# lucasbrynte/gasfm

Hardware: AMD Instinct MI355X
Metric: GAT-stack edges/sec (fwd+bwd) on cam/point scene graph; 1/2/4/8 MI355X (higher is better)
Workload: dtype fp32; 1 GPU; config 4: m=1000 cameras, n=200000 points, E=4001638 projections, 12-block GraphAttnSfMNet (learning_euc widths) fwd+bwd; cameras=1000, points=200000, edges=4001638, blocks=12, parallelism=single GPU

## Files before the change

### gasfm_amd/csrc/global_attn.hip

```cpp
#include <hip/hip_runtime.h>

#include <cstdint>

#include "common.hpp"

namespace gasfm {
namespace {

constexpr int kT = 256;
constexpr int H = 4;
#ifndef GASFM_GATT_CHUNK_V
#define GASFM_GATT_CHUNK_V 8
#endif
#ifndef GASFM_GATT_CHUNK_P
#define GASFM_GATT_CHUNK_P 256
#endif
constexpr int kChunkV = GASFM_GATT_CHUNK_V;
constexpr int kChunkP = GASFM_GATT_CHUNK_P;
constexpr int kMaxProb = 2;
constexpr int kGroup = 32;

struct GaProb {
  const float* XL;
  int64_t ldXL;
  const int32_t* src;
  const float* XR;
  const float* att;
  const float* bias;
  float* out;
  float* smax;
  float* ssum;
  float* part;
  const float* gout;
  float* dXL;
  int64_t ldDXL;
  float* dXR;
  float* datt;
  float* slots;
  uint32_t* cnt;
  int64_t sl;
  int S, HC, C, blk0, nblk;
  float* gslots;
  uint32_t* gcnt;
  int ngroups;
};
struct GaArgs {
  GaProb p[kMaxProb];
  int nprob;
  float slope;
};

__device__ __forceinline__ float leaky(float z, float slope) { return z > 0.f ? z : z * slope; }

__device__ __forceinline__ float wave_sum(float v) {
#pragma unroll
  for (int o = 32; o > 0; o >>= 1) v += __shfl_xor(v, o);
  return v;
}
__device__ __forceinline__ float wave_max(float v) {
#pragma unroll
  for (int o = 32; o > 0; o >>= 1) v = fmaxf(v, __shfl_xor(v, o));
  return v;
}

__device__ __forceinline__ int find_prob(const GaArgs& a) {
  return (a.nprob > 1 && int(blockIdx.x) >= a.p[1].blk0) ? 1 : 0;
}

__device__ __forceinline__ int src_row(const GaProb& p, int j) { return p.src ? p.src[j] : j; }

__device__ __forceinline__ void st_sc1(float* q, float v) {
  __hip_atomic_store(q, v, __ATOMIC_RELAXED, __HIP_MEMORY_SCOPE_AGENT);
}

__device__ __forceinline__ bool last_arrival(uint32_t* cnt, int n, uint32_t* flag) {
  asm volatile("s_waitcnt vmcnt(0)" ::: "memory");
  __syncthreads();
  if (threadIdx.x == 0) {
    const uint32_t t = __hip_atomic_fetch_add(cnt, 1u, __ATOMIC_RELAXED, __HIP_MEMORY_SCOPE_AGENT);
    *flag = t == uint32_t(n - 1) ? 1u : 0u;
  }
  __syncthreads();
  if (*flag == 0u) return false;
  __builtin_amdgcn_fence(__ATOMIC_ACQUIRE, "agent");
  return true;
}

__device__ void merge_fwd(const GaProb& p, float* sc) {
  __shared__ float MH[H], SH[H];
  __shared__ float accg[4][64];
  const int64_t L = p.sl;
  const int n = p.nblk;
  {
    const int h = threadIdx.x & 3;
    float m = -INFINITY;
    for (int k = threadIdx.x >> 2; k < n; k += kT / 4) m = fmaxf(m, p.slots[int64_t(k) * L + p.HC + h]);
#pragma unroll
    for (int o = 32; o >= 4; o >>= 1) m = fmaxf(m, __shfl_xor(m, o));
    __syncthreads();
    if ((threadIdx.x & 63) < 4) sc[(threadIdx.x >> 6) * 4 + h] = m;
    __syncthreads();
    if (threadIdx.x < H)
      MH[threadIdx.x] = fmaxf(fmaxf(sc[threadIdx.x], sc[4 + threadIdx.x]), fmaxf(sc[8 + threadIdx.x], sc[12 + threadIdx.x]));
    __syncthreads();
  }
  {
    const int h = threadIdx.x & 3;
    const float M = MH[h];
    float s = 0.f;
    for (int k = threadIdx.x >> 2; k < n; k += kT / 4) {
      const float* q = p.slots + int64_t(k) * L + p.HC;
      const float mk = q[h], sk = q[H + h];
      s += mk == -INFINITY ? 0.f : sk * __expf(mk - M);
    }
#pragma unroll
    for (int o = 32; o >= 4; o >>= 1) s += __shfl_xor(s, o);
    __syncthreads();
    if ((threadIdx.x & 63) < 4) sc[(threadIdx.x >> 6) * 4 + h] = s;
    __syncthreads();
    if (threadIdx.x < H)
      SH[threadIdx.x] = (sc[threadIdx.x] + sc[4 + threadIdx.x]) + (sc[8 + threadIdx.x] + sc[12 + threadIdx.x]);
    __syncthreads();
  }
  auto finish = [&](int f, float a) {
    const int h = f / p.C;
    if (p.part) {
      st_sc1(p.part + f, a);
      if (f < H) {
        st_sc1(p.part + p.HC + f, MH[f]);
        st_sc1(p.part + p.HC + H + f, SH[f]);
      }
    } else {
      p.out[f] = a / (SH[h] + 1e-16f) + p.bias[f];
      if (f < H) {
        p.smax[f] = MH[f];
        p.ssum[f] = SH[f];
      }
    }
  };
  if (p.C == 256) {
    const int f0 = 4 * threadIdx.x, h = f0 / 256;
    float4 a = make_float4(0.f, 0.f, 0.f, 0.f);
#pragma unroll 8
    for (int k = 0; k < n; ++k) {
      const float* q = p.slots + int64_t(k) * L;
      const float mk = q[p.HC + h];
      const float w = mk == -INFINITY ? 0.f : __expf(mk - MH[h]);
      const float4 v = *reinterpret_cast<const float4*>(q + f0);
      a.x = fmaf(v.x, w, a.x);
      a.y = fmaf(v.y, w, a.y);
      a.z = fmaf(v.z, w, a.z);
      a.w = fmaf(v.w, w, a.w);
    }
    finish(f0, a.x);
    finish(f0 + 1, a.y);
    finish(f0 + 2, a.z);
    finish(f0 + 3, a.w);
  } else {
    const int f = threadIdx.x & 63, grp = threadIdx.x >> 6, h = f / p.C;
    float a = 0.f;
    if (f < p.HC)
#pragma unroll 8
      for (int k = grp; k < n; k += 4) {
        const float* q = p.slots + int64_t(k) * L;
        const float mk = q[p.HC + h];
        a = fmaf(q[f], mk == -INFINITY ? 0.f : __expf(mk - MH[h]), a);
      }
    accg[grp][f] = a;
    __syncthreads();
    if (threadIdx.x < p.HC) finish(threadIdx.x, (accg[0][f] + accg[1][f]) + (accg[2][f] + accg[3][f]));
  }
}

__device__ void done_fwd(const GaProb& p, int blk, uint32_t* flag, float* sc) {
  if (p.ngroups <= 1) {
    if (last_arrival(p.cnt, p.nblk, flag)) {
      merge_fwd(p, sc);
      if (threadIdx.x == 0) __hip_atomic_store(p.cnt, 0u, __ATOMIC_RELAXED, __HIP_MEMORY_SCOPE_AGENT);
    }
    return;
  }
  const int g = blk / kGroup, n0 = g * kGroup;
  const int ng = p.nblk - n0 < kGroup ? p.nblk - n0 : kGroup;
  if (!last_arrival(p.gcnt + g, ng, flag)) return;
  GaProb q = p;
  q.slots = p.slots + int64_t(n0) * p.sl;
  q.nblk = ng;
  q.part = p.gslots + int64_t(g) * p.sl;
  merge_fwd(q, sc);
  if (threadIdx.x == 0) __hip_atomic_store(p.gcnt + g, 0u, __ATOMIC_RELAXED, __HIP_MEMORY_SCOPE_AGENT);
  __syncthreads();
  if (!last_arrival(p.cnt, p.ngroups, flag)) return;
  GaProb r = p;
  r.slots = p.gslots;
  r.nblk = p.ngroups;
  merge_fwd(r, sc);
  if (threadIdx.x == 0) __hip_atomic_store(p.cnt, 0u, __ATOMIC_RELAXED, __HIP_MEMORY_SCOPE_AGENT);
}

__device__ void fwd_views(const GaProb& p, int blk, float slope, uint32_t* flag, float* sc) {
  const int lane = threadIdx.x & 63, wave = threadIdx.x >> 6;
  const int f0 = 4 * threadIdx.x;
  const int j0 = blk * kChunkV, j1 = min(p.S, j0 + kChunkV);
  const float4 xr = *reinterpret_cast<const float4*>(p.XR + f0);
  const float4 at = *reinterpret_cast<const float4*>(p.att + f0);
  float m = -INFINITY, s = 0.f;
  float4 acc = make_float4(0.f, 0.f, 0.f, 0.f);
  float4 nx = make_float4(0.f, 0.f, 0.f, 0.f);
  if (j0 < j1) nx = *reinterpret_cast<const float4*>(p.XL + int64_t(src_row(p, j0)) * p.ldXL + f0);
  for (int j = j0; j < j1; ++j) {
    const float4 x = nx;
    const int jn = j + 1 < j1 ? j + 1 : j;
    nx = *reinterpret_cast<const float4*>(p.XL + int64_t(src_row(p, jn)) * p.ldXL + f0);
    float e = leaky(x.x + xr.x, slope) * at.x + leaky(x.y + xr.y, slope) * at.y + leaky(x.z + xr.z, slope) * at.z +
              leaky(x.w + xr.w, slope) * at.w;
    e = wave_sum(e);
    const float mn = fmaxf(m, e);
    const float sc0 = m == -INFINITY ? 0.f : __expf(m - mn), w = __expf(e - mn);
    s = fmaf(s, sc0, w);
    acc = make_float4(fmaf(acc.x, sc0, w * x.x), fmaf(acc.y, sc0, w * x.y), fmaf(acc.z, sc0, w * x.z),
                      fmaf(acc.w, sc0, w * x.w));
    m = mn;
  }
  float* slot = p.slots + int64_t(blk) * (p.HC + 2 * H);
  st_sc1(slot + f0, acc.x);
  st_sc1(slot + f0 + 1, acc.y);
  st_sc1(slot + f0 + 2, acc.z);
  st_sc1(slot + f0 + 3, acc.w);
  if (lane == 0) {
    st_sc1(slot + p.HC + wave, m);
    st_sc1(slot + p.HC + H + wave, s);
  }
  done_fwd(p, blk, flag, sc);
}

__device__ void fwd_points(const GaProb& p, int blk, float slope, uint32_t* flag, float* sc) {
  __shared__ float SM[16][H], SS[16][H];
  __shared__ float4 SA[16][16];
  const int ql = threadIdx.x >> 4, fq = threadIdx.x & 15, h = fq >> 2;
  const int f0 = 4 * fq;
  const int j0 = blk * kChunkP, j1 = min(p.S, j0 + kChunkP);
  const float4 xr = *reinterpret_cast<const float4*>(p.XR + f0);
  const float4 at = *reinterpret_cast<const float4*>(p.att + f0);
  float m = -INFINITY, s = 0.f;
  float4 acc = make_float4(0.f, 0.f, 0.f, 0.f);
  constexpr int U = 4;
  for (int jb = j0 + ql; jb < j1; jb += 16 * U) {
    float4 x[U];
#pragma unroll
    for (int u = 0; u < U; ++u) {
      const int j = jb + 16 * u;
      x[u] = *reinterpret_cast<const float4*>(p.XL + int64_t(src_row(p, j < j1 ? j : jb)) * p.ldXL + f0);
    }
#pragma unroll
    for (int u = 0; u < U; ++u) {
      float e = leaky(x[u].x + xr.x, slope) * at.x + leaky(x[u].y + xr.y, slope) * at.y +
                leaky(x[u].z + xr.z, slope) * at.z + leaky(x[u].w + xr.w, slope) * at.w;
      e += __shfl_xor(e, 1);
      e += __shfl_xor(e, 2);
      if (jb + 16 * u < j1) {
        const float mn = fmaxf(m, e);
        const float sc0 = m == -INFINITY ? 0.f : __expf(m - mn), w = __expf(e - mn);
        s = fmaf(s, sc0, w);
        acc = make_float4(fmaf(acc.x, sc0, w * x[u].x), fmaf(acc.y, sc0, w * x[u].y), fmaf(acc.z, sc0, w * x[u].z),
                          fmaf(acc.w, sc0, w * x[u].w));
        m = mn;
      }
    }
  }
  if ((fq & 3) == 0) {
    SM[ql][h] = m;
    SS[ql][h] = s;
  }
  SA[ql][fq] = acc;
  __syncthreads();
  float* slot = p.slots + int64_t(blk) * (p.HC + 2 * H);
  if (threadIdx.x < 16) {
    const int hh = threadIdx.x >> 2;
    float M = -INFINITY;
#pragma unroll
    for (int q = 0; q < 16; ++q) M = fmaxf(M, SM[q][hh]);
    float S = 0.f;
    float4 A = make_float4(0.f, 0.f, 0.f, 0.f);
#pragma unroll
    for (int q = 0; q < 16; ++q) {
      const float mq = SM[q][hh];
      const float w = mq == -INFINITY ? 0.f : __expf(mq - M);
      S = fmaf(SS[q][hh], w, S);
      const float4 a = SA[q][threadIdx.x];
      A = make_float4(fmaf(a.x, w, A.x), fmaf(a.y, w, A.y), fmaf(a.z, w, A.z), fmaf(a.w, w, A.w));
    }
    const int g0 = 4 * threadIdx.x;
    st_sc1(slot + g0, A.x);
    st_sc1(slot + g0 + 1, A.y);
    st_sc1(slot + g0 + 2, A.z);
    st_sc1(slot + g0 + 3, A.w);
    if ((threadIdx.x & 3) == 0) {
      st_sc1(slot + p.HC + hh, M);
      st_sc1(slot + p.HC + H + hh, S);
    }
  }
  done_fwd(p, blk, flag, sc);
}

__global__ __launch_bounds__(kT) void gatt_fwd_kernel(GaArgs a) {
  __shared__ uint32_t flag;
  __shared__ float sc[16];
  const int pi = find_prob(a);
  const GaProb& p = a.p[pi];
  const int blk = int(blockIdx.x) - p.blk0;
  if (p.C == 256)
    fwd_views(p, blk, a.slope, &flag, sc);
  else
    fwd_points(p, blk, a.slope, &flag, sc);
}

__device__ void merge_bwd(const GaProb& p, bool final = true, float* grow = nullptr) {
  __shared__ float acc4[4][2 * 64];
  const int L = 2 * p.HC, n = p.nblk;
  if (p.C == 256) {
    for (int half = 0; half < 2; ++half) {
      const int f0 = 4 * threadIdx.x;
      float4 a = make_float4(0.f, 0.f, 0.f, 0.f);
#pragma unroll 8
      for (int k = 0; k < n; ++k) {
        const float4 v = *reinterpret_cast<const float4*>(p.slots + int64_t(k) * L + half * p.HC + f0);
        a.x += v.x;
        a.y += v.y;
        a.z += v.z;
        a.w += v.w;
      }
      if (!final) {
        float* d = grow + half * p.HC + f0;
        st_sc1(d, a.x);
        st_sc1(d + 1, a.y);
        st_sc1(d + 2, a.z);
        st_sc1(d + 3, a.w);
        continue;
      }
      float* d = half ? p.datt : p.dXR;
      d[f0] = a.x;
      d[f0 + 1] = a.y;
      d[f0 + 2] = a.z;
      d[f0 + 3] = a.w;
    }
    if (final)
      *reinterpret_cast<float4*>(p.datt + p.HC + 4 * threadIdx.x) =
          *reinterpret_cast<const float4*>(p.gout + 4 * threadIdx.x);
  } else {
    const int grp = threadIdx.x >> 6;
#pragma unroll
    for (int r = 0; r < 2; ++r) {
      const int v = (threadIdx.x & 63) + 64 * r;
      float a = 0.f;
      if (v < L)
#pragma unroll 8
        for (int k = grp; k < n; k += 4) a += p.slots[int64_t(k) * L + v];
      acc4[grp][v] = a;
    }
    __syncthreads();
    if (threadIdx.x < L) {
      const float a = (acc4[0][threadIdx.x] + acc4[1][threadIdx.x]) + (acc4[2][threadIdx.x] + acc4[3][threadIdx.x]);
      if (!final)
        st_sc1(grow + threadIdx.x, a);
      else if (threadIdx.x < p.HC)
        p.dXR[threadIdx.x] = a;
      else
        p.datt[threadIdx.x - p.HC] = a;
    }
    if (final && threadIdx.x < p.HC) p.datt[p.HC + threadIdx.x] = p.gout[threadIdx.x];
  }
}

__device__ void done_bwd(const GaProb& p, int blk, uint32_t* flag) {
  if (p.ngroups <= 1) {
    if (last_arrival(p.cnt, p.nblk, flag)) {
      merge_bwd(p);
      if (threadIdx.x == 0) __hip_atomic_store(p.cnt, 0u, __ATOMIC_RELAXED, __HIP_MEMORY_SCOPE_AGENT);
    }
    return;
  }
  const int g = blk / kGroup, n0 = g * kGroup;
  const int ng = p.nblk - n0 < kGroup ? p.nblk - n0 : kGroup;
  if (!last_arrival(p.gcnt + g, ng, flag)) return;
  const int64_t L = 2 * int64_t(p.HC);
  GaProb q = p;
  q.slots = p.slots + int64_t(n0) * L;
  q.nblk = ng;
  merge_bwd(q, false, p.gslots + int64_t(g) * L);
  if (threadIdx.x == 0) __hip_atomic_store(p.gcnt + g, 0u, __ATOMIC_RELAXED, __HIP_MEMORY_SCOPE_AGENT);
  __syncthreads();
  if (!last_arrival(p.cnt, p.ngroups, flag)) return;
  GaProb r = p;
  r.slots = p.gslots;
  r.nblk = p.ngroups;
  merge_bwd(r);
  if (threadIdx.x == 0) __hip_atomic_store(p.cnt, 0u, __ATOMIC_RELAXED, __HIP_MEMORY_SCOPE_AGENT);
}

__device__ void bwd_views(const GaProb& p, int blk, float slope, uint32_t* flag) {
  const int lane = threadIdx.x & 63, wave = threadIdx.x >> 6;
  const int f0 = 4 * threadIdx.x;
  const int j0 = blk * kChunkV, j1 = min(p.S, j0 + kChunkV);
  const float4 xr = *reinterpret_cast<const float4*>(p.XR + f0);
  const float4 at = *reinterpret_cast<const float4*>(p.att + f0);
  const float4 go = *reinterpret_cast<const float4*>(p.gout + f0);
  const float4 o4 = *reinterpret_cast<const float4*>(p.out + f0);
  const float4 b4 = *reinterpret_cast<const float4*>(p.bias + f0);
  const float M = p.smax[wave], inv = 1.f / (p.ssum[wave] + 1e-16f);
  const float delta =
      wave_sum(go.x * (o4.x - b4.x) + go.y * (o4.y - b4.y) + go.z * (o4.z - b4.z) + go.w * (o4.w - b4.w));
  float4 dxr = make_float4(0.f, 0.f, 0.f, 0.f), dat = dxr;
  int jr = 0;
  float4 nx = make_float4(0.f, 0.f, 0.f, 0.f);
  if (j0 < j1) {
    jr = src_row(p, j0);
    nx = *reinterpret_cast<const float4*>(p.XL + int64_t(jr) * p.ldXL + f0);
  }
  for (int j = j0; j < j1; ++j) {
    const float4 x = nx;
    const int row = jr;
    const int jn = j + 1 < j1 ? j + 1 : j;
    jr = src_row(p, jn);
    nx = *reinterpret_cast<const float4*>(p.XL + int64_t(jr) * p.ldXL + f0);
    const float z[4] = {x.x + xr.x, x.y + xr.y, x.z + xr.z, x.w + xr.w};
    const float a4[4] = {at.x, at.y, at.z, at.w};
    const float g4[4] = {go.x, go.y, go.z, go.w};
    const float xv[4] = {x.x, x.y, x.z, x.w};
    float e = 0.f, da = 0.f;
#pragma unroll
    for (int k = 0; k < 4; ++k) {
      e = fmaf(leaky(z[k], slope), a4[k], e);
      da = fmaf(g4[k], xv[k], da);
    }
    e = wave_sum(e);
    da = wave_sum(da);
    const float alpha = __expf(e - M) * inv;
    const float de = alpha * (da - delta);
    float dxl[4], dz[4];
#pragma unroll
    for (int k = 0; k < 4; ++k) {
      dz[k] = de * a4[k] * (z[k] > 0.f ? 1.f : slope);
      dxl[k] = fmaf(alpha, g4[k], dz[k]);
    }
    *reinterpret_cast<float4*>(p.dXL + int64_t(row) * p.ldDXL + f0) = make_float4(dxl[0], dxl[1], dxl[2], dxl[3]);
    dxr = make_float4(dxr.x + dz[0], dxr.y + dz[1], dxr.z + dz[2], dxr.w + dz[3]);
    dat = make_float4(fmaf(de, leaky(z[0], slope), dat.x), fmaf(de, leaky(z[1], slope), dat.y),
                      fmaf(de, leaky(z[2], slope), dat.z), fmaf(de, leaky(z[3], slope), dat.w));
  }
  float* slot = p.slots + int64_t(blk) * 2 * p.HC;
  st_sc1(slot + f0, dxr.x);
  st_sc1(slot + f0 + 1, dxr.y);
  st_sc1(slot + f0 + 2, dxr.z);
  st_sc1(slot + f0 + 3, dxr.w);
  st_sc1(slot + p.HC + f0, dat.x);
  st_sc1(slot + p.HC + f0 + 1, dat.y);
  st_sc1(slot + p.HC + f0 + 2, dat.z);
  st_sc1(slot + p.HC + f0 + 3, dat.w);
  (void)lane;
  done_bwd(p, blk, flag);
}

__device__ void bwd_points(const GaProb& p, int blk, float slope, uint32_t* flag) {
  __shared__ float4 SX[16][16], SD[16][16];
  const int ql = threadIdx.x >> 4, fq = threadIdx.x & 15, h = fq >> 2;
  const int f0 = 4 * fq;
  const int j0 = blk * kChunkP, j1 = min(p.S, j0 + kChunkP);
  const float4 xr = *reinterpret_cast<const float4*>(p.XR + f0);
  const float4 at = *reinterpret_cast<const float4*>(p.att + f0);
  const float4 go = *reinterpret_cast<const float4*>(p.gout + f0);
  const float4 o4 = *reinterpret_cast<const float4*>(p.out + f0);
  const float4 b4 = *reinterpret_cast<const float4*>(p.bias + f0);
  const float M = p.smax[h], inv = 1.f / (p.ssum[h] + 1e-16f);
  float delta = go.x * (o4.x - b4.x) + go.y * (o4.y - b4.y) + go.z * (o4.z - b4.z) + go.w * (o4.w - b4.w);
  delta += __shfl_xor(delta, 1);
  delta += __shfl_xor(delta, 2);
  const float a4[4] = {at.x, at.y, at.z, at.w};
  const float g4[4] = {go.x, go.y, go.z, go.w};
  float4 dxr = make_float4(0.f, 0.f, 0.f, 0.f), dat = dxr;
  constexpr int U = 4;
  for (int jb = j0 + ql; jb < j1; jb += 16 * U) {
    float4 x[U];
    int rows[U];
#pragma unroll
    for (int u = 0; u < U; ++u) {
      const int j = jb + 16 * u;
      rows[u] = src_row(p, j < j1 ? j : jb);
      x[u] = *reinterpret_cast<const float4*>(p.XL + int64_t(rows[u]) * p.ldXL + f0);
    }
#pragma unroll
    for (int u = 0; u < U; ++u) {
      const float xv[4] = {x[u].x, x[u].y, x[u].z, x[u].w};
      float z[4], e = 0.f, da = 0.f;
#pragma unroll
      for (int k = 0; k < 4; ++k) {
        z[k] = xv[k] + (k == 0 ? xr.x : k == 1 ? xr.y : k == 2 ? xr.z : xr.w);
        e = fmaf(leaky(z[k], slope), a4[k], e);
        da = fmaf(g4[k], xv[k], da);
      }
      e += __shfl_xor(e, 1);
      e += __shfl_xor(e, 2);
      da += __shfl_xor(da, 1);
      da += __shfl_xor(da, 2);
      if (jb + 16 * u < j1) {
        const float alpha = __expf(e - M) * inv;
        const float de = alpha * (da - delta);
        float dxl[4];
#pragma unroll
        for (int k = 0; k < 4; ++k) {
          const float dz = de * a4[k] * (z[k] > 0.f ? 1.f : slope);
          dxl[k] = fmaf(alpha, g4[k], dz);
          if (k == 0) dxr.x += dz, dat.x = fmaf(de, leaky(z[k], slope), dat.x);
          if (k == 1) dxr.y += dz, dat.y = fmaf(de, leaky(z[k], slope), dat.y);
          if (k == 2) dxr.z += dz, dat.z = fmaf(de, leaky(z[k], slope), dat.z);
          if (k == 3) dxr.w += dz, dat.w = fmaf(de, leaky(z[k], slope), dat.w);
        }
        *reinterpret_cast<float4*>(p.dXL + int64_t(rows[u]) * p.ldDXL + f0) =
            make_float4(dxl[0], dxl[1], dxl[2], dxl[3]);
      }
    }
  }
  SX[ql][fq] = dxr;
  SD[ql][fq] = dat;
  __syncthreads();
  float* slot = p.slots + int64_t(blk) * 2 * p.HC;
  if (threadIdx.x < 32) {
    const int q = threadIdx.x & 15, half = threadIdx.x >> 4;
    float4 sum = make_float4(0.f, 0.f, 0.f, 0.f);
#pragma unroll
    for (int l = 0; l < 16; ++l) {
      const float4 v = half ? SD[l][q] : SX[l][q];
      sum = make_float4(sum.x + v.x, sum.y + v.y, sum.z + v.z, sum.w + v.w);
    }
    float* d = slot + half * p.HC + 4 * q;
    st_sc1(d, sum.x);
    st_sc1(d + 1, sum.y);
    st_sc1(d + 2, sum.z);
    st_sc1(d + 3, sum.w);
  }
  done_bwd(p, blk, flag);
}

__global__ __launch_bounds__(kT) void gatt_bwd_kernel(GaArgs a) {
  __shared__ uint32_t flag;
  const int pi = find_prob(a);
  const GaProb& p = a.p[pi];
  const int blk = int(blockIdx.x) - p.blk0;
  if (p.C == 256)
    bwd_views(p, blk, a.slope, &flag);
  else
    bwd_points(p, blk, a.slope, &flag);
}

struct Unpack {
  const float* G;
  int64_t blk, roff, soff, ld_dst;
  float* rows_dst;
  float* sum_dst;
  int W, chunk, width, m, sn;
};

__device__ __forceinline__ int unpack_units(const Unpack& u) {
  return (u.rows_dst ? u.m * (u.width / 4) : 0) + (u.sum_dst ? u.sn / 4 : 0);
}

__device__ __forceinline__ void unpack_unit(const Unpack& u, int k) {
  const int nr = u.rows_dst ? u.m * (u.width / 4) : 0;
  if (k < nr) {
    const int w4 = u.width / 4, c = k / w4, q = k % w4;
    const float4 v = *reinterpret_cast<const float4*>(u.G + int64_t(c / u.chunk) * u.blk + u.roff +
                                                      int64_t(c % u.chunk) * u.width + 4 * q);
    *reinterpret_cast<float4*>(u.rows_dst + int64_t(c) * u.ld_dst + 4 * q) = v;
    return;
  }
  const int j = k - nr;
  float4 acc = *reinterpret_cast<const float4*>(u.G + u.soff + 4 * j);
  for (int r = 1; r < u.W; ++r) {
    const float4 v = *reinterpret_cast<const float4*>(u.G + int64_t(r) * u.blk + u.soff + 4 * j);
    acc = make_float4(acc.x + v.x, acc.y + v.y, acc.z + v.z, acc.w + v.w);
  }
  *reinterpret_cast<float4*>(u.sum_dst + 4 * j) = acc;
}

__global__ __launch_bounds__(kT) void exchange_unpack_kernel(Unpack u) {
  const int k = int(blockIdx.x) * kT + int(threadIdx.x);
  if (k < unpack_units(u)) unpack_unit(u, k);
}

__global__ __launch_bounds__(kT) void gatt_merge_kernel(GaArgs a, Unpack u) {
  __shared__ float sc[16];
  if (int(blockIdx.x) < a.nprob) {
    merge_fwd(a.p[blockIdx.x], sc);
    return;
  }
  const int k = (int(blockIdx.x) - a.nprob) * kT + int(threadIdx.x);
  if (k < unpack_units(u)) unpack_unit(u, k);
}

int chunk_of(int C) { return C == 256 ? kChunkV : kChunkP; }

int groups_of(int nblk) { return nblk > kGroup ? (nblk + kGroup - 1) / kGroup : 1; }

int setup(const gasfm_gatt_prob* in, int nprob, float* scratch, uint32_t* counters, bool bwd, GaArgs& a) {
  a.nprob = nprob;
  int blocks = 0;
  float* ws = scratch;
  uint32_t* cn = counters;
  for (int q = 0; q < nprob; ++q) {
    const gasfm_gatt_prob& s = in[q];
    GaProb& p = a.p[q];
    p.XL = s.XL, p.ldXL = s.ldXL, p.src = s.src, p.XR = s.XR, p.att = s.att, p.bias = s.bias;
    p.out = s.out, p.smax = s.smax, p.ssum = s.ssum, p.part = s.part;
    p.gout = s.gout, p.dXL = s.dXL, p.ldDXL = s.ldDXL, p.dXR = s.dXR, p.datt = s.datt;
    p.S = s.S, p.HC = s.HC, p.C = s.HC / H;
    p.nblk = (s.S + chunk_of(p.C) - 1) / chunk_of(p.C);
    if (p.nblk < 1) p.nblk = 1;
    p.blk0 = blocks;
    p.slots = ws;
    p.sl = p.HC + 2 * H;
    const int64_t slot = bwd ? 2 * p.HC : p.HC + 2 * H;
    ws += int64_t(p.nblk) * slot;
    p.ngroups = groups_of(p.nblk);
    p.gslots = ws;
    if (p.ngroups > 1) ws += int64_t(p.ngroups) * slot;
    p.cnt = cn++;
    p.gcnt = cn;
    if (p.ngroups > 1) cn += p.ngroups;
    blocks += p.nblk;
  }
  for (int q = nprob; q < kMaxProb; ++q) a.p[q].blk0 = blocks;
  return blocks;
}

}
}

using namespace gasfm;

static int gatt_check(int32_t nprob, const gasfm_gatt_prob* probs, bool bwd) {
  GASFM_REQUIRE(nprob >= 1 && nprob <= kMaxProb && probs, "gasfm_gatt: nprob=%d", nprob);
  for (int q = 0; q < nprob; ++q) {
    const gasfm_gatt_prob& p = probs[q];
    GASFM_REQUIRE(p.HC == 4 * 256 || p.HC == 4 * 16, "gasfm_gatt: problem %d HC=%d (H = 4, C in {16, 256})", q, p.HC);
    GASFM_REQUIRE(p.S >= 0 && (p.XL || p.S == 0) && p.XR && p.att && p.bias && p.ldXL % 4 == 0 && (p.ldXL >= p.HC || p.S == 0),
                  "gasfm_gatt: problem %d S=%d / pointers / ldXL", q, p.S);
    GASFM_REQUIRE(aligned16(p.XL) && aligned16(p.XR) && aligned16(p.att) && aligned16(p.bias),
                  "gasfm_gatt: problem %d alignment", q);
    if (!bwd) {
      GASFM_REQUIRE(p.part || (p.out && p.smax && p.ssum), "gasfm_gatt_fwd: problem %d outputs", q);
    } else {
      GASFM_REQUIRE(p.gout && p.out && p.smax && p.ssum && (p.dXL || p.S == 0) && p.dXR && p.datt && p.ldDXL % 4 == 0 &&
                        (aligned16(p.dXL) || p.S == 0) && aligned16(p.gout) && aligned16(p.out) && aligned16(p.datt),
                    "gasfm_gatt_bwd: problem %d pointers", q);
    }
  }
  return GASFM_OK;
}

static int64_t nblk_of(const gasfm_gatt_prob& p) {
  const int C = p.HC / H;
  const int64_t nblk = (p.S + chunk_of(C) - 1) / chunk_of(C);
  return nblk < 1 ? 1 : nblk;
}

extern "C" int64_t gasfm_gatt_scratch_floats(int32_t nprob, const gasfm_gatt_prob* probs) {
  int64_t n = 0;
  for (int q = 0; q < nprob; ++q) {
    const int64_t nblk = nblk_of(probs[q]), ng = groups_of(int(nblk));
    n += (nblk + (ng > 1 ? ng : 0)) * (2 * int64_t(probs[q].HC) + 2 * H);
  }
  return n + 16;
}

extern "C" int32_t gasfm_gatt_counters(int32_t nprob, const gasfm_gatt_prob* probs) {
  int32_t n = 0;
  for (int q = 0; q < nprob; ++q) {
    const int ng = groups_of(int(nblk_of(probs[q])));
    n += 1 + (ng > 1 ? ng : 0);
  }
  return n;
}

extern "C" int gasfm_gatt_fwd(int32_t nprob, const gasfm_gatt_prob* probs, float slope, float* scratch,
                              uint32_t* counters, void* stream) {
  const int s0 = gatt_check(nprob, probs, false);
  if (s0 != GASFM_OK) return s0;
  GASFM_REQUIRE(scratch && counters, "gasfm_gatt_fwd: scratch / counters");
  GaArgs a{};
  a.slope = slope;
  const int blocks = setup(probs, nprob, scratch, counters, false, a);
  hipLaunchKernelGGL(gatt_fwd_kernel, dim3(blocks), dim3(kT), 0, reinterpret_cast<hipStream_t>(stream), a);
  return launch_status("gasfm_gatt_fwd");
}

static int unpack_check(const Unpack& u, const char* who) {
  GASFM_REQUIRE(u.G && u.W >= 1 && u.blk % 4 == 0 && u.roff % 4 == 0 && u.soff % 4 == 0 && u.width % 4 == 0 &&
                    u.ld_dst % 4 == 0 && u.sn % 4 == 0 && u.m >= 0 && u.chunk >= 1 && u.m <= int64_t(u.W) * u.chunk &&
                    aligned16(u.G) && aligned16(u.rows_dst) && aligned16(u.sum_dst) &&
                    (!u.rows_dst || (u.roff + int64_t(u.chunk) * u.width <= u.blk && u.ld_dst >= u.width)) &&
                    (!u.sum_dst || u.soff + u.sn <= u.blk),
                "%s: W=%d blk=%lld roff=%lld chunk=%d width=%d m=%d soff=%lld sn=%d (layout / alignment)", who, u.W,
                (long long)u.blk, (long long)u.roff, u.chunk, u.width, u.m, (long long)u.soff, u.sn);
  return GASFM_OK;
}

static Unpack make_unpack(const float* G, int32_t W, int64_t blk, int64_t roff, int32_t chunk, int32_t width, int32_t m,
                          float* rows_dst, int64_t ld_dst, int64_t soff, int32_t sn, float* sum_dst) {
  Unpack u;
  u.G = G, u.blk = blk, u.roff = roff, u.soff = soff, u.ld_dst = ld_dst;
  u.rows_dst = rows_dst, u.sum_dst = sum_dst;
  u.W = W, u.chunk = chunk, u.width = width, u.m = m, u.sn = sn;
  return u;
}

extern "C" int gasfm_exchange_unpack(const float* G, int32_t W, int64_t blk, int64_t roff, int32_t chunk,
                                     int32_t width, int32_t m, float* rows_dst, int64_t ld_dst, int64_t soff,
                                     int32_t sn, float* sum_dst, void* stream) {
  const Unpack u = make_unpack(G, W, blk, roff, chunk, width, m, rows_dst, ld_dst, soff, sn, sum_dst);
  const int s0 = unpack_check(u, "gasfm_exchange_unpack");
  if (s0 != GASFM_OK) return s0;
  const int units = (rows_dst ? m * (width / 4) : 0) + (sum_dst ? sn / 4 : 0);
  if (units == 0) return GASFM_OK;
  hipLaunchKernelGGL(exchange_unpack_kernel, dim3((units + kT - 1) / kT), dim3(kT), 0,
                     reinterpret_cast<hipStream_t>(stream), u);
  return launch_status("gasfm_exchange_unpack");
}

static int merge_launch(int32_t nprob, const gasfm_gatt_prob* probs, int32_t nrows, int64_t stride, const Unpack& u,
                        void* stream);

extern "C" int gasfm_gatt_merge(int32_t nprob, const gasfm_gatt_prob* probs, int32_t nrows, int64_t stride,
                                void* stream) {
  Unpack u{};
  return merge_launch(nprob, probs, nrows, stride, u, stream);
}

extern "C" int gasfm_gatt_merge_unpack(int32_t nprob, const gasfm_gatt_prob* probs, int32_t nrows, int64_t stride,
                                       const float* G, int32_t W, int64_t blk, int64_t roff, int32_t chunk,
                                       int32_t width, int32_t m, float* rows_dst, int64_t ld_dst, void* stream) {
  GASFM_REQUIRE(rows_dst, "gasfm_gatt_merge_unpack: rows_dst");
  const Unpack u = make_unpack(G, W, blk, roff, chunk, width, m, rows_dst, ld_dst, 0, 0, nullptr);
  const int s0 = unpack_check(u, "gasfm_gatt_merge_unpack");
  if (s0 != GASFM_OK) return s0;
  return merge_launch(nprob, probs, nrows, stride, u, stream);
}

static int merge_launch(int32_t nprob, const gasfm_gatt_prob* probs, int32_t nrows, int64_t stride, const Unpack& u,
                        void* stream) {
  GASFM_REQUIRE(nprob >= 1 && nprob <= kMaxProb && probs && nrows >= 1, "gasfm_gatt_merge: nprob=%d nrows=%d", nprob,
                nrows);
  GaArgs a{};
  a.nprob = nprob;
  for (int q = 0; q < nprob; ++q) {
    const gasfm_gatt_prob& s = probs[q];
    GASFM_REQUIRE((s.HC == 1024 || s.HC == 64) && s.part && s.bias && s.out && s.smax && s.ssum &&
                      stride >= s.HC + 2 * H,
                  "gasfm_gatt_merge: problem %d HC=%d / pointers / stride", q, s.HC);
    GaProb& p = a.p[q];
    p.HC = s.HC, p.C = s.HC / H, p.bias = s.bias, p.out = s.out, p.smax = s.smax, p.ssum = s.ssum;
    p.part = nullptr;
    p.slots = const_cast<float*>(s.part);
    p.sl = stride;
    p.nblk = nrows;
    p.ngroups = 1;
  }
  const int units = u.G ? (u.rows_dst ? u.m * (u.width / 4) : 0) + (u.sum_dst ? u.sn / 4 : 0) : 0;
  hipLaunchKernelGGL(gatt_merge_kernel, dim3(nprob + (units + kT - 1) / kT), dim3(kT), 0,
                     reinterpret_cast<hipStream_t>(stream), a, u);
  return launch_status("gasfm_gatt_merge");
}

extern "C" int gasfm_gatt_bwd(int32_t nprob, const gasfm_gatt_prob* probs, float slope, float* scratch,
                              uint32_t* counters, void* stream) {
  const int s0 = gatt_check(nprob, probs, true);
  if (s0 != GASFM_OK) return s0;
  GASFM_REQUIRE(scratch && counters, "gasfm_gatt_bwd: scratch / counters");
  GaArgs a{};
  a.slope = slope;
  const int blocks = setup(probs, nprob, scratch, counters, true, a);
  hipLaunchKernelGGL(gatt_bwd_kernel, dim3(blocks), dim3(kT), 0, reinterpret_cast<hipStream_t>(stream), a);
  return launch_status("gasfm_gatt_bwd");
}
```

Baseline: 144.5 million edges/s.

## Restructure global attention into occupancy-capped ranges with batched online softmax

Replaces the fixed-chunk view and point kernels with one templated range kernel. Each block now processes a contiguous range sized from the resident-block count, with a cap on slots. Rows are prefetched kDepth at a time with double buffering, and the online-softmax rescale happens once per batch instead of once per row. The two-level group merge is removed because fewer slots need merging, and the merges are vectorised with float4. The cost targeted is merge and atomic overhead plus memory latency. In exchange, the path depends on occupancy queries and uses more registers.

```diff
diff --git a/gasfm_amd/csrc/global_attn.hip b/gasfm_amd/csrc/global_attn.hip
--- a/gasfm_amd/csrc/global_attn.hip
+++ b/gasfm_amd/csrc/global_attn.hip
@@ -10,15 +10,30 @@
 constexpr int kT = 256;
 constexpr int H = 4;
 #ifndef GASFM_GATT_CHUNK_V
-#define GASFM_GATT_CHUNK_V 8
+#define GASFM_GATT_CHUNK_V 16
 #endif
-#ifndef GASFM_GATT_CHUNK_P
-#define GASFM_GATT_CHUNK_P 256
+#ifndef GASFM_GATT_MIN_RANGE_P
+#define GASFM_GATT_MIN_RANGE_P 256
+#endif
+#ifndef GASFM_GATT_MAX_SLOTS_FWD
+#define GASFM_GATT_MAX_SLOTS_FWD 256
+#endif
+#ifndef GASFM_GATT_MAX_SLOTS_BWD
+#define GASFM_GATT_MAX_SLOTS_BWD 512
+#endif
+#ifndef GASFM_GATT_DEPTH
+#define GASFM_GATT_DEPTH 8
 #endif
 constexpr int kChunkV = GASFM_GATT_CHUNK_V;
-constexpr int kChunkP = GASFM_GATT_CHUNK_P;
+constexpr int kMinRangeP = GASFM_GATT_MIN_RANGE_P;
+constexpr int kMaxSlotsFwd = GASFM_GATT_MAX_SLOTS_FWD;
+constexpr int kMaxSlotsBwd = GASFM_GATT_MAX_SLOTS_BWD;
+constexpr int kMaxSlots = kMaxSlotsFwd > kMaxSlotsBwd ? kMaxSlotsFwd : kMaxSlotsBwd;
+constexpr int kDepth = GASFM_GATT_DEPTH;
 constexpr int kMaxProb = 2;
-constexpr int kGroup = 32;
+constexpr int kShared4 = 512;
+
+typedef float v4f __attribute__((ext_vector_type(4)));
 
 struct GaProb {
   const float* XL;
@@ -40,9 +55,7 @@
   uint32_t* cnt;
   int64_t sl;
   int S, HC, C, blk0, nblk;
-  float* gslots;
-  uint32_t* gcnt;
-  int ngroups;
+  int range;
 };
 struct GaArgs {
   GaProb p[kMaxProb];
@@ -57,9 +70,12 @@
   for (int o = 32; o > 0; o >>= 1) v += __shfl_xor(v, o);
   return v;
 }
-__device__ __forceinline__ float wave_max(float v) {
-#pragma unroll
-  for (int o = 32; o > 0; o >>= 1) v = fmaxf(v, __shfl_xor(v, o));
+
+template <int C>
+__device__ __forceinline__ float head_sum(float v) {
+  if (C == 256) return wave_sum(v);
+  v += __shfl_xor(v, 1);
+  v += __shfl_xor(v, 2);
   return v;
 }
 
@@ -67,10 +83,30 @@
   return (a.nprob > 1 && int(blockIdx.x) >= a.p[1].blk0) ? 1 : 0;
 }
 
-__device__ __forceinline__ int src_row(const GaProb& p, int j) { return p.src ? p.src[j] : j; }
-
 __device__ __forceinline__ void st_sc1(float* q, float v) {
   __hip_atomic_store(q, v, __ATOMIC_RELAXED, __HIP_MEMORY_SCOPE_AGENT);
+}
+
+__device__ __forceinline__ float4 f4zero() { return make_float4(0.f, 0.f, 0.f, 0.f); }
+__device__ __forceinline__ float4 f4add(float4 a, float4 b) {
+  return make_float4(a.x + b.x, a.y + b.y, a.z + b.z, a.w + b.w);
+}
+__device__ __forceinline__ float4 f4fma(float4 v, float w, float4 a) {
+  return make_float4(fmaf(v.x, w, a.x), fmaf(v.y, w, a.y), fmaf(v.z, w, a.z), fmaf(v.w, w, a.w));
+}
+
+template <bool SRC>
+__device__ __forceinline__ void row_ids(const GaProb& p, int j0, int step, int jl, int (&r)[kDepth]) {
+#pragma unroll
+  for (int u = 0; u < kDepth; ++u) {
+    const int j = min(j0 + step * u, jl);
+    r[u] = SRC ? p.src[j] : j;
+  }
+}
+
+__device__ __forceinline__ void load_rows(const GaProb& p, const int (&r)[kDepth], int f0, float4 (&x)[kDepth]) {
+#pragma unroll
+  for (int u = 0; u < kDepth; ++u) x[u] = *reinterpret_cast<const float4*>(p.XL + int64_t(r[u]) * p.ldXL + f0);
 }
 
 __device__ __forceinline__ bool last_arrival(uint32_t* cnt, int n, uint32_t* flag) {
@@ -86,14 +122,17 @@
   return true;
 }
 
-__device__ void merge_fwd(const GaProb& p, float* sc) {
-  __shared__ float MH[H], SH[H];
-  __shared__ float accg[4][64];
+__device__ void merge_fwd(const GaProb& p, float4* sh) {
+  float* MH = reinterpret_cast<float*>(sh);
+  float* SH = MH + H;
+  float* sc = MH + 2 * H;
+  float4* accg = sh + 8;
   const int64_t L = p.sl;
   const int n = p.nblk;
   {
     const int h = threadIdx.x & 3;
     float m = -INFINITY;
+#pragma unroll 4
     for (int k = threadIdx.x >> 2; k < n; k += kT / 4) m = fmaxf(m, p.slots[int64_t(k) * L + p.HC + h]);
 #pragma unroll
     for (int o = 32; o >= 4; o >>= 1) m = fmaxf(m, __shfl_xor(m, o));
@@ -108,6 +147,7 @@
     const int h = threadIdx.x & 3;
     const float M = MH[h];
     float s = 0.f;
+#pragma unroll 4
     for (int k = threadIdx.x >> 2; k < n; k += kT / 4) {
       const float* q = p.slots + int64_t(k) * L + p.HC;
       const float mk = q[h], sk = q[H + h];
@@ -122,434 +162,352 @@
       SH[threadIdx.x] = (sc[threadIdx.x] + sc[4 + threadIdx.x]) + (sc[8 + threadIdx.x] + sc[12 + threadIdx.x]);
     __syncthreads();
   }
-  auto finish = [&](int f, float a) {
-    const int h = f / p.C;
+  auto finish = [&](int f0, float4 a) {
+    const int h = f0 / p.C;
     if (p.part) {
-      st_sc1(p.part + f, a);
-      if (f < H) {
-        st_sc1(p.part + p.HC + f, MH[f]);
-        st_sc1(p.part + p.HC + H + f, SH[f]);
+      *reinterpret_cast<float4*>(p.part + f0) = a;
+      if (f0 == 0) {
+        *reinterpret_cast<float4*>(p.part + p.HC) = make_float4(MH[0], MH[1], MH[2], MH[3]);
+        *reinterpret_cast<float4*>(p.part + p.HC + H) = make_float4(SH[0], SH[1], SH[2], SH[3]);
       }
     } else {
-      p.out[f] = a / (SH[h] + 1e-16f) + p.bias[f];
-      if (f < H) {
-        p.smax[f] = MH[f];
-        p.ssum[f] = SH[f];
-      }
+      const float inv = SH[h] + 1e-16f;
+      p.out[f0] = a.x / inv + p.bias[f0];
+      p.out[f0 + 1] = a.y / inv + p.bias[f0 + 1];
+      p.out[f0 + 2] = a.z / inv + p.bias[f0 + 2];
+      p.out[f0 + 3] = a.w / inv + p.bias[f0 + 3];
+      if (f0 == 0)
+        for (int i = 0; i < H; ++i) {
+          p.smax[i] = MH[i];
+          p.ssum[i] = SH[i];
+        }
     }
   };
   if (p.C == 256) {
     const int f0 = 4 * threadIdx.x, h = f0 / 256;
-    float4 a = make_float4(0.f, 0.f, 0.f, 0.f);
-#pragma unroll 8
+    const float Mh = MH[h];
+    float4 a = f4zero();
+#pragma unroll 16
     for (int k = 0; k < n; ++k) {
       const float* q = p.slots + int64_t(k) * L;
       const float mk = q[p.HC + h];
-      const float w = mk == -INFINITY ? 0.f : __expf(mk - MH[h]);
       const float4 v = *reinterpret_cast<const float4*>(q + f0);
-      a.x = fmaf(v.x, w, a.x);
-      a.y = fmaf(v.y, w, a.y);
-      a.z = fmaf(v.z, w, a.z);
-      a.w = fmaf(v.w, w, a.w);
-    }
-    finish(f0, a.x);
-    finish(f0 + 1, a.y);
-    finish(f0 + 2, a.z);
-    finish(f0 + 3, a.w);
+      a = f4fma(v, mk == -INFINITY ? 0.f : __expf(mk - Mh), a);
+    }
+    finish(f0, a);
   } else {
-    const int f = threadIdx.x & 63, grp = threadIdx.x >> 6, h = f / p.C;
-    float a = 0.f;
-    if (f < p.HC)
+    const int q4 = threadIdx.x & 15, g = threadIdx.x >> 4, h = q4 >> 2;
+    const float Mh = MH[h];
+    float4 a = f4zero();
 #pragma unroll 8
-      for (int k = grp; k < n; k += 4) {
-        const float* q = p.slots + int64_t(k) * L;
-        const float mk = q[p.HC + h];
-        a = fmaf(q[f], mk == -INFINITY ? 0.f : __expf(mk - MH[h]), a);
-      }
-    accg[grp][f] = a;
-    __syncthreads();
-    if (threadIdx.x < p.HC) finish(threadIdx.x, (accg[0][f] + accg[1][f]) + (accg[2][f] + accg[3][f]));
-  }
-}
-
-__device__ void done_fwd(const GaProb& p, int blk, uint32_t* flag, float* sc) {
-  if (p.ngroups <= 1) {
-    if (last_arrival(p.cnt, p.nblk, flag)) {
-      merge_fwd(p, sc);
-      if (threadIdx.x == 0) __hip_atomic_store(p.cnt, 0u, __ATOMIC_RELAXED, __HIP_MEMORY_SCOPE_AGENT);
-    }
-    return;
-  }
-  const int g = blk / kGroup, n0 = g * kGroup;
-  const int ng = p.nblk - n0 < kGroup ? p.nblk - n0 : kGroup;
-  if (!last_arrival(p.gcnt + g, ng, flag)) return;
-  GaProb q = p;
-  q.slots = p.slots + int64_t(n0) * p.sl;
-  q.nblk = ng;
-  q.part = p.gslots + int64_t(g) * p.sl;
-  merge_fwd(q, sc);
-  if (threadIdx.x == 0) __hip_atomic_store(p.gcnt + g, 0u, __ATOMIC_RELAXED, __HIP_MEMORY_SCOPE_AGENT);
-  __syncthreads();
-  if (!last_arrival(p.cnt, p.ngroups, flag)) return;
-  GaProb r = p;
-  r.slots = p.gslots;
-  r.nblk = p.ngroups;
-  merge_fwd(r, sc);
-  if (threadIdx.x == 0) __hip_atomic_store(p.cnt, 0u, __ATOMIC_RELAXED, __HIP_MEMORY_SCOPE_AGENT);
-}
-
-__device__ void fwd_views(const GaProb& p, int blk, float slope, uint32_t* flag, float* sc) {
-  const int lane = threadIdx.x & 63, wave = threadIdx.x >> 6;
-  const int f0 = 4 * threadIdx.x;
-  const int j0 = blk * kChunkV, j1 = min(p.S, j0 + kChunkV);
+    for (int k = g; k < n; k += 16) {
+      const float* q = p.slots + int64_t(k) * L;
+      const float mk = q[p.HC + h];
+      const float4 v = *reinterpret_cast<const float4*>(q + 4 * q4);
+      a = f4fma(v, mk == -INFINITY ? 0.f : __expf(mk - Mh), a);
+    }
+    accg[g * 16 + q4] = a;
+    __syncthreads();
+    if (threadIdx.x < 16) {
+      float4 t = accg[threadIdx.x];
+#pragma unroll
+      for (int i = 1; i < 16; ++i) t = f4add(t, accg[i * 16 + threadIdx.x]);
+      finish(4 * threadIdx.x, t);
+    }
+  }
+}
+
+__device__ void done_fwd(const GaProb& p, uint32_t* flag, float4* sh) {
+  if (last_arrival(p.cnt, p.nblk, flag)) {
+    merge_fwd(p, sh);
+    if (threadIdx.x == 0) __hip_atomic_store(p.cnt, 0u, __ATOMIC_RELAXED, __HIP_MEMORY_SCOPE_AGENT);
+  }
+}
+
+template <int C, bool SRC>
+__device__ void fwd_range(const GaProb& p, int blk, float slope, uint32_t* flag, float4* sh) {
+  constexpr int kStep = C == 16 ? 16 : 1;
+  constexpr int kSpan = kStep * kDepth;
+  const int ql = C == 16 ? int(threadIdx.x >> 4) : 0;
+  const int fq = C == 16 ? int(threadIdx.x & 15) : int(threadIdx.x);
+  const int f0 = 4 * fq;
+  const int r0 = int(min(int64_t(p.S), int64_t(blk) * p.range)), r1 = int(min(int64_t(p.S), int64_t(r0) + p.range));
   const float4 xr = *reinterpret_cast<const float4*>(p.XR + f0);
   const float4 at = *reinterpret_cast<const float4*>(p.att + f0);
   float m = -INFINITY, s = 0.f;
-  float4 acc = make_float4(0.f, 0.f, 0.f, 0.f);
-  float4 nx = make_float4(0.f, 0.f, 0.f, 0.f);
-  if (j0 < j1) nx = *reinterpret_cast<const float4*>(p.XL + int64_t(src_row(p, j0)) * p.ldXL + f0);
-  for (int j = j0; j < j1; ++j) {
-    const float4 x = nx;
-    const int jn = j + 1 < j1 ? j + 1 : j;
-    nx = *reinterpret_cast<const float4*>(p.XL + int64_t(src_row(p, jn)) * p.ldXL + f0);
-    float e = leaky(x.x + xr.x, slope) * at.x + leaky(x.y + xr.y, slope) * at.y + leaky(x.z + xr.z, slope) * at.z +
-              leaky(x.w + xr.w, slope) * at.w;
-    e = wave_sum(e);
-    const float mn = fmaxf(m, e);
-    const float sc0 = m == -INFINITY ? 0.f : __expf(m - mn), w = __expf(e - mn);
-    s = fmaf(s, sc0, w);
-    acc = make_float4(fmaf(acc.x, sc0, w * x.x), fmaf(acc.y, sc0, w * x.y), fmaf(acc.z, sc0, w * x.z),
-                      fmaf(acc.w, sc0, w * x.w));
-    m = mn;
+  float4 acc = f4zero();
+  if (r0 < r1) {
+    const int jl = r1 - 1;
+    const int nb = (r1 - r0 + kSpan - 1) / kSpan;
+    auto consume = [&](const float4(&x)[kDepth], int jb) {
+      float e[kDepth];
+      float mb = m;
+#pragma unroll
+      for (int u = 0; u < kDepth; ++u) {
+        float t = leaky(x[u].x + xr.x, slope) * at.x + leaky(x[u].y + xr.y, slope) * at.y +
+                  leaky(x[u].z + xr.z, slope) * at.z + leaky(x[u].w + xr.w, slope) * at.w;
+        t = head_sum<C>(t);
+        e[u] = jb + kStep * u < r1 ? t : -INFINITY;
+        mb = fmaxf(mb, e[u]);
+      }
+      const float sc0 = m == -INFINITY ? 0.f : __expf(m - mb);
+      s *= sc0;
+      acc = make_float4(acc.x * sc0, acc.y * sc0, acc.z * sc0, acc.w * sc0);
+#pragma unroll
+      for (int u = 0; u < kDepth; ++u) {
+        const float w = e[u] == -INFINITY ? 0.f : __expf(e[u] - mb);
+        s += w;
+        acc = f4fma(x[u], w, acc);
+      }
+      m = mb;
+    };
+    int iA[kDepth], iB[kDepth];
+    float4 A[kDepth], B[kDepth];
+    const int j0 = r0 + ql;
+    row_ids<SRC>(p, j0, kStep, jl, iA);
+    load_rows(p, iA, f0, A);
+    row_ids<SRC>(p, j0 + kSpan, kStep, jl, iB);
+    for (int b = 0; b < nb; b += 2) {
+      const int jb = j0 + b * kSpan;
+      load_rows(p, iB, f0, B);
+      __builtin_amdgcn_sched_barrier(0);
+      consume(A, jb);
+      row_ids<SRC>(p, jb + 2 * kSpan, kStep, jl, iA);
+      load_rows(p, iA, f0, A);
+      __builtin_amdgcn_sched_barrier(0);
+      consume(B, jb + kSpan);
+      row_ids<SRC>(p, jb + 3 * kSpan, kStep, jl, iB);
+    }
   }
   float* slot = p.slots + int64_t(blk) * (p.HC + 2 * H);
-  st_sc1(slot + f0, acc.x);
-  st_sc1(slot + f0 + 1, acc.y);
-  st_sc1(slot + f0 + 2, acc.z);
-  st_sc1(slot + f0 + 3, acc.w);
-  if (lane == 0) {
-    st_sc1(slot + p.HC + wave, m);
-    st_sc1(slot + p.HC + H + wave, s);
-  }
-  done_fwd(p, blk, flag, sc);
-}
-
-__device__ void fwd_points(const GaProb& p, int blk, float slope, uint32_t* flag, float* sc) {
-  __shared__ float SM[16][H], SS[16][H];
-  __shared__ float4 SA[16][16];
-  const int ql = threadIdx.x >> 4, fq = threadIdx.x & 15, h = fq >> 2;
-  const int f0 = 4 * fq;
-  const int j0 = blk * kChunkP, j1 = min(p.S, j0 + kChunkP);
-  const float4 xr = *reinterpret_cast<const float4*>(p.XR + f0);
-  const float4 at = *reinterpret_cast<const float4*>(p.att + f0);
-  float m = -INFINITY, s = 0.f;
-  float4 acc = make_float4(0.f, 0.f, 0.f, 0.f);
-  constexpr int U = 4;
-  for (int jb = j0 + ql; jb < j1; jb += 16 * U) {
-    float4 x[U];
-#pragma unroll
-    for (int u = 0; u < U; ++u) {
-      const int j = jb + 16 * u;
-      x[u] = *reinterpret_cast<const float4*>(p.XL + int64_t(src_row(p, j < j1 ? j : jb)) * p.ldXL + f0);
-    }
-#pragma unroll
-    for (int u = 0; u < U; ++u) {
-      float e = leaky(x[u].x + xr.x, slope) * at.x + leaky(x[u].y + xr.y, slope) * at.y +
-                leaky(x[u].z + xr.z, slope) * at.z + leaky(x[u].w + xr.w, slope) * at.w;
-      e += __shfl_xor(e, 1);
-      e += __shfl_xor(e, 2);
-      if (jb + 16 * u < j1) {
-        const float mn = fmaxf(m, e);
-        const float sc0 = m == -INFINITY ? 0.f : __expf(m - mn), w = __expf(e - mn);
-        s = fmaf(s, sc0, w);
-        acc = make_float4(fmaf(acc.x, sc0, w * x[u].x), fmaf(acc.y, sc0, w * x[u].y), fmaf(acc.z, sc0, w * x[u].z),
-                          fmaf(acc.w, sc0, w * x[u].w));
-        m = mn;
+  if (C == 256) {
+    const int lane = threadIdx.x & 63, wave = threadIdx.x >> 6;
+    st_sc1(slot + f0, acc.x);
+    st_sc1(slot + f0 + 1, acc.y);
+    st_sc1(slot + f0 + 2, acc.z);
+    st_sc1(slot + f0 + 3, acc.w);
+    if (lane == 0) {
+      st_sc1(slot + p.HC + wave, m);
+      st_sc1(slot + p.HC + H + wave, s);
+    }
+  } else {
+    float4* SA = sh;
+    float* SM = reinterpret_cast<float*>(sh + 256);
+    float* SS = SM + 16 * H;
+    const int h = fq >> 2;
+    if ((fq & 3) == 0) {
+      SM[ql * H + h] = m;
+      SS[ql * H + h] = s;
+    }
+    SA[ql * 16 + fq] = acc;
+    __syncthreads();
+    if (threadIdx.x < 16) {
+      const int hh = threadIdx.x >> 2;
+      float M = -INFINITY;
+#pragma unroll
+      for (int q = 0; q < 16; ++q) M = fmaxf(M, SM[q * H + hh]);
+      float S = 0.f;
+      float4 A = f4zero();
+#pragma unroll
+      for (int q = 0; q < 16; ++q) {
+        const float mq = SM[q * H + hh];
+        const float w = mq == -INFINITY ? 0.f : __expf(mq - M);
+        S = fmaf(SS[q * H + hh], w, S);
+        A = f4fma(SA[q * 16 + threadIdx.x], w, A);
       }
-    }
-  }
-  if ((fq & 3) == 0) {
-    SM[ql][h] = m;
-    SS[ql][h] = s;
-  }
-  SA[ql][fq] = acc;
-  __syncthreads();
-  float* slot = p.slots + int64_t(blk) * (p.HC + 2 * H);
-  if (threadIdx.x < 16) {
-    const int hh = threadIdx.x >> 2;
-    float M = -INFINITY;
-#pragma unroll
-    for (int q = 0; q < 16; ++q) M = fmaxf(M, SM[q][hh]);
-    float S = 0.f;
-    float4 A = make_float4(0.f, 0.f, 0.f, 0.f);
-#pragma unroll
-    for (int q = 0; q < 16; ++q) {
-      const float mq = SM[q][hh];
-      const float w = mq == -INFINITY ? 0.f : __expf(mq - M);
-      S = fmaf(SS[q][hh], w, S);
-      const float4 a = SA[q][threadIdx.x];
-      A = make_float4(fmaf(a.x, w, A.x), fmaf(a.y, w, A.y), fmaf(a.z, w, A.z), fmaf(a.w, w, A.w));
-    }
-    const int g0 = 4 * threadIdx.x;
-    st_sc1(slot + g0, A.x);
-    st_sc1(slot + g0 + 1, A.y);
-    st_sc1(slot + g0 + 2, A.z);
-    st_sc1(slot + g0 + 3, A.w);
-    if ((threadIdx.x & 3) == 0) {
-      st_sc1(slot + p.HC + hh, M);
-      st_sc1(slot + p.HC + H + hh, S);
-    }
-  }
-  done_fwd(p, blk, flag, sc);
+      const int g0 = 4 * threadIdx.x;
+      st_sc1(slot + g0, A.x);
+      st_sc1(slot + g0 + 1, A.y);
+      st_sc1(slot + g0 + 2, A.z);
+      st_sc1(slot + g0 + 3, A.w);
+      if ((threadIdx.x & 3) == 0) {
+        st_sc1(slot + p.HC + hh, M);
+        st_sc1(slot + p.HC + H + hh, S);
+      }
+    }
+  }
+  done_fwd(p, flag, sh);
 }
 
 __global__ __launch_bounds__(kT) void gatt_fwd_kernel(GaArgs a) {
   __shared__ uint32_t flag;
-  __shared__ float sc[16];
+  __shared__ float4 sh[kShared4];
   const int pi = find_prob(a);
   const GaProb& p = a.p[pi];
   const int blk = int(blockIdx.x) - p.blk0;
-  if (p.C == 256)
-    fwd_views(p, blk, a.slope, &flag, sc);
-  else
-    fwd_points(p, blk, a.slope, &flag, sc);
-}
-
-__device__ void merge_bwd(const GaProb& p, bool final = true, float* grow = nullptr) {
-  __shared__ float acc4[4][2 * 64];
+  if (p.C == 256) {
+    if (p.src)
+      fwd_range<256, true>(p, blk, a.slope, &flag, sh);
+    else
+      fwd_range<256, false>(p, blk, a.slope, &flag, sh);
+  } else {
+    if (p.src)
+      fwd_range<16, true>(p, blk, a.slope, &flag, sh);
+    else
+      fwd_range<16, false>(p, blk, a.slope, &flag, sh);
+  }
+}
+
+__device__ void merge_bwd(const GaProb& p, float4* sh) {
   const int L = 2 * p.HC, n = p.nblk;
   if (p.C == 256) {
-    for (int half = 0; half < 2; ++half) {
+    const int f0 = 4 * threadIdx.x;
+    float4 a = f4zero(), b = f4zero();
+#pragma unroll 8
+    for (int k = 0; k < n; ++k) {
+      const float* q = p.slots + int64_t(k) * L + f0;
+      a = f4add(a, *reinterpret_cast<const float4*>(q));
+      b = f4add(b, *reinterpret_cast<const float4*>(q + p.HC));
+    }
+    *reinterpret_cast<float4*>(p.dXR + f0) = a;
+    *reinterpret_cast<float4*>(p.datt + f0) = b;
+    *reinterpret_cast<float4*>(p.datt + p.HC + f0) = *reinterpret_cast<const float4*>(p.gout + f0);
+  } else {
+    const int q4 = threadIdx.x & 31, g = threadIdx.x >> 5;
+    float4 a = f4zero();
+#pragma unroll 8
+    for (int k = g; k < n; k += 8) a = f4add(a, *reinterpret_cast<const float4*>(p.slots + int64_t(k) * L + 4 * q4));
+    sh[g * 32 + q4] = a;
+    __syncthreads();
+    if (threadIdx.x < 32) {
+      float4 t = sh[threadIdx.x];
+#pragma unroll
+      for (int i = 1; i < 8; ++i) t = f4add(t, sh[i * 32 + threadIdx.x]);
       const int f0 = 4 * threadIdx.x;
-      float4 a = make_float4(0.f, 0.f, 0.f, 0.f);
-#pragma unroll 8
-      for (int k = 0; k < n; ++k) {
-        const float4 v = *reinterpret_cast<const float4*>(p.slots + int64_t(k) * L + half * p.HC + f0);
-        a.x += v.x;
-        a.y += v.y;
-        a.z += v.z;
-        a.w += v.w;
+      if (f0 < p.HC) {
+        *reinterpret_cast<float4*>(p.dXR + f0) = t;
+        *reinterpret_cast<float4*>(p.datt + p.HC + f0) = *reinterpret_cast<const float4*>(p.gout + f0);
+      } else {
+        *reinterpret_cast<float4*>(p.datt + f0 - p.HC) = t;
       }
-      if (!final) {
-        float* d = grow + half * p.HC + f0;
-        st_sc1(d, a.x);
-        st_sc1(d + 1, a.y);
-        st_sc1(d + 2, a.z);
-        st_sc1(d + 3, a.w);
-        continue;
-      }
-      float* d = half ? p.datt : p.dXR;
-      d[f0] = a.x;
-      d[f0 + 1] = a.y;
-      d[f0 + 2] = a.z;
-      d[f0 + 3] = a.w;
-    }
-    if (final)
-      *reinterpret_cast<float4*>(p.datt + p.HC + 4 * threadIdx.x) =
-          *reinterpret_cast<const float4*>(p.gout + 4 * threadIdx.x);
-  } else {
-    const int grp = threadIdx.x >> 6;
-#pragma unroll
-    for (int r = 0; r < 2; ++r) {
-      const int v = (threadIdx.x & 63) + 64 * r;
-      float a = 0.f;
-      if (v < L)
-#pragma unroll 8
-        for (int k = grp; k < n; k += 4) a += p.slots[int64_t(k) * L + v];
-      acc4[grp][v] = a;
-    }
-    __syncthreads();
-    if (threadIdx.x < L) {
-      const float a = (acc4[0][threadIdx.x] + acc4[1][threadIdx.x]) + (acc4[2][threadIdx.x] + acc4[3][threadIdx.x]);
-      if (!final)
-        st_sc1(grow + threadIdx.x, a);
-      else if (threadIdx.x < p.HC)
-        p.dXR[threadIdx.x] = a;
-      else
-        p.datt[threadIdx.x - p.HC] = a;
-    }
-    if (final && threadIdx.x < p.HC) p.datt[p.HC + threadIdx.x] = p.gout[threadIdx.x];
-  }
-}
-
-__device__ void done_bwd(const GaProb& p, int blk, uint32_t* flag) {
-  if (p.ngroups <= 1) {
-    if (last_arrival(p.cnt, p.nblk, flag)) {
-      merge_bwd(p);
-      if (threadIdx.x == 0) __hip_atomic_store(p.cnt, 0u, __ATOMIC_RELAXED, __HIP_MEMORY_SCOPE_AGENT);
-    }
-    return;
-  }
-  const int g = blk / kGroup, n0 = g * kGroup;
-  const int ng = p.nblk - n0 < kGroup ? p.nblk - n0 : kGroup;
-  if (!last_arrival(p.gcnt + g, ng, flag)) return;
-  const int64_t L = 2 * int64_t(p.HC);
-  GaProb q = p;
-  q.slots = p.slots + int64_t(n0) * L;
-  q.nblk = ng;
-  merge_bwd(q, false, p.gslots + int64_t(g) * L);
-  if (threadIdx.x == 0) __hip_atomic_store(p.gcnt + g, 0u, __ATOMIC_RELAXED, __HIP_MEMORY_SCOPE_AGENT);
-  __syncthreads();
-  if (!last_arrival(p.cnt, p.ngroups, flag)) return;
-  GaProb r = p;
-  r.slots = p.gslots;
-  r.nblk = p.ngroups;
-  merge_bwd(r);
-  if (threadIdx.x == 0) __hip_atomic_store(p.cnt, 0u, __ATOMIC_RELAXED, __HIP_MEMORY_SCOPE_AGENT);
-}
-
-__device__ void bwd_views(const GaProb& p, int blk, float slope, uint32_t* flag) {
-  const int lane = threadIdx.x & 63, wave = threadIdx.x >> 6;
-  const int f0 = 4 * threadIdx.x;
-  const int j0 = blk * kChunkV, j1 = min(p.S, j0 + kChunkV);
-  const float4 xr = *reinterpret_cast<const float4*>(p.XR + f0);
-  const float4 at = *reinterpret_cast<const float4*>(p.att + f0);
-  const float4 go = *reinterpret_cast<const float4*>(p.gout + f0);
-  const float4 o4 = *reinterpret_cast<const float4*>(p.out + f0);
-  const float4 b4 = *reinterpret_cast<const float4*>(p.bias + f0);
-  const float M = p.smax[wave], inv = 1.f / (p.ssum[wave] + 1e-16f);
-  const float delta =
-      wave_sum(go.x * (o4.x - b4.x) + go.y * (o4.y - b4.y) + go.z * (o4.z - b4.z) + go.w * (o4.w - b4.w));
-  float4 dxr = make_float4(0.f, 0.f, 0.f, 0.f), dat = dxr;
-  int jr = 0;
-  float4 nx = make_float4(0.f, 0.f, 0.f, 0.f);
-  if (j0 < j1) {
-    jr = src_row(p, j0);
-    nx = *reinterpret_cast<const float4*>(p.XL + int64_t(jr) * p.ldXL + f0);
-  }
-  for (int j = j0; j < j1; ++j) {
-    const float4 x = nx;
-    const int row = jr;
-    const int jn = j + 1 < j1 ? j + 1 : j;
-    jr = src_row(p, jn);
-    nx = *reinterpret_cast<const float4*>(p.XL + int64_t(jr) * p.ldXL + f0);
-    const float z[4] = {x.x + xr.x, x.y + xr.y, x.z + xr.z, x.w + xr.w};
-    const float a4[4] = {at.x, at.y, at.z, at.w};
-    const float g4[4] = {go.x, go.y, go.z, go.w};
-    const float xv[4] = {x.x, x.y, x.z, x.w};
-    float e = 0.f, da = 0.f;
-#pragma unroll
-    for (int k = 0; k < 4; ++k) {
-      e = fmaf(leaky(z[k], slope), a4[k], e);
-      da = fmaf(g4[k], xv[k], da);
-    }
-    e = wave_sum(e);
-    da = wave_sum(da);
-    const float alpha = __expf(e - M) * inv;
-    const float de = alpha * (da - delta);
-    float dxl[4], dz[4];
-#pragma unroll
-    for (int k = 0; k < 4; ++k) {
-      dz[k] = de * a4[k] * (z[k] > 0.f ? 1.f : slope);
-      dxl[k] = fmaf(alpha, g4[k], dz[k]);
-    }
-    *reinterpret_cast<float4*>(p.dXL + int64_t(row) * p.ldDXL + f0) = make_float4(dxl[0], dxl[1], dxl[2], dxl[3]);
-    dxr = make_float4(dxr.x + dz[0], dxr.y + dz[1], dxr.z + dz[2], dxr.w + dz[3]);
-    dat = make_float4(fmaf(de, leaky(z[0], slope), dat.x), fmaf(de, leaky(z[1], slope), dat.y),
-                      fmaf(de, leaky(z[2], slope), dat.z), fmaf(de, leaky(z[3], slope), dat.w));
-  }
-  float* slot = p.slots + int64_t(blk) * 2 * p.HC;
-  st_sc1(slot + f0, dxr.x);
-  st_sc1(slot + f0 + 1, dxr.y);
-  st_sc1(slot + f0 + 2, dxr.z);
-  st_sc1(slot + f0 + 3, dxr.w);
-  st_sc1(slot + p.HC + f0, dat.x);
-  st_sc1(slot + p.HC + f0 + 1, dat.y);
-  st_sc1(slot + p.HC + f0 + 2, dat.z);
-  st_sc1(slot + p.HC + f0 + 3, dat.w);
-  (void)lane;
-  done_bwd(p, blk, flag);
-}
-
-__device__ void bwd_points(const GaProb& p, int blk, float slope, uint32_t* flag) {
-  __shared__ float4 SX[16][16], SD[16][16];
-  const int ql = threadIdx.x >> 4, fq = threadIdx.x & 15, h = fq >> 2;
+    }
+  }
+}
+
+__device__ void done_bwd(const GaProb& p, uint32_t* flag, float4* sh) {
+  if (last_arrival(p.cnt, p.nblk, flag)) {
+    merge_bwd(p, sh);
+    if (threadIdx.x == 0) __hip_atomic_store(p.cnt, 0u, __ATOMIC_RELAXED, __HIP_MEMORY_SCOPE_AGENT);
+  }
+}
+
+template <int C, bool SRC>
+__device__ void bwd_range(const GaProb& p, int blk, float slope, uint32_t* flag, float4* sh) {
+  constexpr int kStep = C == 16 ? 16 : 1;
+  constexpr int kSpan = kStep * kDepth;
+  const int ql = C == 16 ? int(threadIdx.x >> 4) : 0;
+  const int fq = C == 16 ? int(threadIdx.x & 15) : int(threadIdx.x);
   const int f0 = 4 * fq;
-  const int j0 = blk * kChunkP, j1 = min(p.S, j0 + kChunkP);
+  const int h = C == 16 ? fq >> 2 : int(threadIdx.x >> 6);
+  const int r0 = int(min(int64_t(p.S), int64_t(blk) * p.range)), r1 = int(min(int64_t(p.S), int64_t(r0) + p.range));
   const float4 xr = *reinterpret_cast<const float4*>(p.XR + f0);
   const float4 at = *reinterpret_cast<const float4*>(p.att + f0);
   const float4 go = *reinterpret_cast<const float4*>(p.gout + f0);
   const float4 o4 = *reinterpret_cast<const float4*>(p.out + f0);
   const float4 b4 = *reinterpret_cast<const float4*>(p.bias + f0);
   const float M = p.smax[h], inv = 1.f / (p.ssum[h] + 1e-16f);
-  float delta = go.x * (o4.x - b4.x) + go.y * (o4.y - b4.y) + go.z * (o4.z - b4.z) + go.w * (o4.w - b4.w);
-  delta += __shfl_xor(delta, 1);
-  delta += __shfl_xor(delta, 2);
+  const float delta =
+      head_sum<C>(go.x * (o4.x - b4.x) + go.y * (o4.y - b4.y) + go.z * (o4.z - b4.z) + go.w * (o4.w - b4.w));
+  const float xr4[4] = {xr.x, xr.y, xr.z, xr.w};
   const float a4[4] = {at.x, at.y, at.z, at.w};
   const float g4[4] = {go.x, go.y, go.z, go.w};
-  float4 dxr = make_float4(0.f, 0.f, 0.f, 0.f), dat = dxr;
-  constexpr int U = 4;
-  for (int jb = j0 + ql; jb < j1; jb += 16 * U) {
-    float4 x[U];
-    int rows[U];
-#pragma unroll
-    for (int u = 0; u < U; ++u) {
-      const int j = jb + 16 * u;
-      rows[u] = src_row(p, j < j1 ? j : jb);
-      x[u] = *reinterpret_cast<const float4*>(p.XL + int64_t(rows[u]) * p.ldXL + f0);
-    }
-#pragma unroll
-    for (int u = 0; u < U; ++u) {
-      const float xv[4] = {x[u].x, x[u].y, x[u].z, x[u].w};
-      float z[4], e = 0.f, da = 0.f;
-#pragma unroll
-      for (int k = 0; k < 4; ++k) {
-        z[k] = xv[k] + (k == 0 ? xr.x : k == 1 ? xr.y : k == 2 ? xr.z : xr.w);
-        e = fmaf(leaky(z[k], slope), a4[k], e);
-        da = fmaf(g4[k], xv[k], da);
-      }
-      e += __shfl_xor(e, 1);
-      e += __shfl_xor(e, 2);
-      da += __shfl_xor(da, 1);
-      da += __shfl_xor(da, 2);
-      if (jb + 16 * u < j1) {
-        const float alpha = __expf(e - M) * inv;
+  float dxr[4] = {0.f, 0.f, 0.f, 0.f}, dat[4] = {0.f, 0.f, 0.f, 0.f};
+  if (r0 < r1) {
+    const int jl = r1 - 1;
+    const int nb = (r1 - r0 + kSpan - 1) / kSpan;
+    auto consume = [&](const float4(&x)[kDepth], const int(&rows)[kDepth], int jb) {
+#pragma unroll
+      for (int u = 0; u < kDepth; ++u) {
+        const float xv[4] = {x[u].x, x[u].y, x[u].z, x[u].w};
+        float z[4], e = 0.f, da = 0.f;
+#pragma unroll
+        for (int k = 0; k < 4; ++k) {
+          z[k] = xv[k] + xr4[k];
+          e = fmaf(leaky(z[k], slope), a4[k], e);
+          da = fmaf(g4[k], xv[k], da);
+        }
+        e = head_sum<C>(e);
+        da = head_sum<C>(da);
+        const bool live = jb + kStep * u < r1;
+        const float alpha = live ? __expf(e - M) * inv : 0.f;
         const float de = alpha * (da - delta);
         float dxl[4];
 #pragma unroll
         for (int k = 0; k < 4; ++k) {
           const float dz = de * a4[k] * (z[k] > 0.f ? 1.f : slope);
           dxl[k] = fmaf(alpha, g4[k], dz);
-          if (k == 0) dxr.x += dz, dat.x = fmaf(de, leaky(z[k], slope), dat.x);
-          if (k == 1) dxr.y += dz, dat.y = fmaf(de, leaky(z[k], slope), dat.y);
-          if (k == 2) dxr.z += dz, dat.z = fmaf(de, leaky(z[k], slope), dat.z);
-          if (k == 3) dxr.w += dz, dat.w = fmaf(de, leaky(z[k], slope), dat.w);
+          dxr[k] += dz;
+          dat[k] = fmaf(de, leaky(z[k], slope), dat[k]);
         }
-        *reinterpret_cast<float4*>(p.dXL + int64_t(rows[u]) * p.ldDXL + f0) =
-            make_float4(dxl[0], dxl[1], dxl[2], dxl[3]);
+        if (live)
+          __builtin_nontemporal_store(v4f{dxl[0], dxl[1], dxl[2], dxl[3]},
+                                      reinterpret_cast<v4f*>(p.dXL + int64_t(rows[u]) * p.ldDXL + f0));
       }
-    }
-  }
-  SX[ql][fq] = dxr;
-  SD[ql][fq] = dat;
-  __syncthreads();
+    };
+    int iA[kDepth], iB[kDepth];
+    float4 A[kDepth], B[kDepth];
+    const int j0 = r0 + ql;
+    row_ids<SRC>(p, j0, kStep, jl, iA);
+    load_rows(p, iA, f0, A);
+    row_ids<SRC>(p, j0 + kSpan, kStep, jl, iB);
+    for (int b = 0; b < nb; b += 2) {
+      const int jb = j0 + b * kSpan;
+      load_rows(p, iB, f0, B);
+      __builtin_amdgcn_sched_barrier(0);
+      consume(A, iA, jb);
+      row_ids<SRC>(p, jb + 2 * kSpan, kStep, jl, iA);
+      load_rows(p, iA, f0, A);
+      __builtin_amdgcn_sched_barrier(0);
+      consume(B, iB, jb + kSpan);
+      row_ids<SRC>(p, jb + 3 * kSpan, kStep, jl, iB);
+    }
+  }
   float* slot = p.slots + int64_t(blk) * 2 * p.HC;
-  if (threadIdx.x < 32) {
-    const int q = threadIdx.x & 15, half = threadIdx.x >> 4;
-    float4 sum = make_float4(0.f, 0.f, 0.f, 0.f);
-#pragma unroll
-    for (int l = 0; l < 16; ++l) {
-      const float4 v = half ? SD[l][q] : SX[l][q];
-      sum = make_float4(sum.x + v.x, sum.y + v.y, sum.z + v.z, sum.w + v.w);
-    }
-    float* d = slot + half * p.HC + 4 * q;
-    st_sc1(d, sum.x);
-    st_sc1(d + 1, sum.y);
-    st_sc1(d + 2, sum.z);
-    st_sc1(d + 3, sum.w);
-  }
-  done_bwd(p, blk, flag);
+  if (C == 256) {
+#pragma unroll
+    for (int k = 0; k < 4; ++k) {
+      st_sc1(slot + f0 + k, dxr[k]);
+      st_sc1(slot + p.HC + f0 + k, dat[k]);
+    }
+  } else {
+    float4* SX = sh;
+    float4* SD = sh + 256;
+    SX[ql * 16 + fq] = make_float4(dxr[0], dxr[1], dxr[2], dxr[3]);
+    SD[ql * 16 + fq] = make_float4(dat[0], dat[1], dat[2], dat[3]);
+    __syncthreads();
+    if (threadIdx.x < 32) {
+      const int q = threadIdx.x & 15, half = threadIdx.x >> 4;
+      const float4* src = half ? SD : SX;
+      float4 sum = f4zero();
+#pragma unroll
+      for (int l = 0; l < 16; ++l) sum = f4add(sum, src[l * 16 + q]);
+      float* d = slot + half * p.HC + 4 * q;
+      st_sc1(d, sum.x);
+      st_sc1(d + 1, sum.y);
+      st_sc1(d + 2, sum.z);
+      st_sc1(d + 3, sum.w);
+    }
+  }
+  done_bwd(p, flag, sh);
 }
 
 __global__ __launch_bounds__(kT) void gatt_bwd_kernel(GaArgs a) {
   __shared__ uint32_t flag;
+  __shared__ float4 sh[kShared4];
   const int pi = find_prob(a);
   const GaProb& p = a.p[pi];
   const int blk = int(blockIdx.x) - p.blk0;
-  if (p.C == 256)
-    bwd_views(p, blk, a.slope, &flag);
-  else
-    bwd_points(p, blk, a.slope, &flag);
+  if (p.C == 256) {
+    if (p.src)
+      bwd_range<256, true>(p, blk, a.slope, &flag, sh);
+    else
+      bwd_range<256, false>(p, blk, a.slope, &flag, sh);
+  } else {
+    if (p.src)
+      bwd_range<16, true>(p, blk, a.slope, &flag, sh);
+    else
+      bwd_range<16, false>(p, blk, a.slope, &flag, sh);
+  }
 }
 
 struct Unpack {
@@ -588,21 +546,35 @@
 }
 
 __global__ __launch_bounds__(kT) void gatt_merge_kernel(GaArgs a, Unpack u) {
-  __shared__ float sc[16];
+  __shared__ float4 sh[kShared4];
   if (int(blockIdx.x) < a.nprob) {
-    merge_fwd(a.p[blockIdx.x], sc);
+    merge_fwd(a.p[blockIdx.x], sh);
     return;
   }
   const int k = (int(blockIdx.x) - a.nprob) * kT + int(threadIdx.x);
   if (k < unpack_units(u)) unpack_unit(u, k);
 }
 
-int chunk_of(int C) { return C == 256 ? kChunkV : kChunkP; }
-
-int groups_of(int nblk) { return nblk > kGroup ? (nblk + kGroup - 1) / kGroup : 1; }
+int range_of(int S, int G) {
+  const int r = (S + G - 1) / G;
+  return r < 16 ? 16 : (r + 15) / 16 * 16;
+}
+
+int blocks_of(int S, int C, int cap) {
+  if (C == 256) return S > kChunkV ? (S + kChunkV - 1) / kChunkV : 1;
+  const int64_t want = (int64_t(S) + kMinRangeP - 1) / kMinRangeP;
+  return int(want < 1 ? 1 : (want > cap ? cap : want));
+}
 
 int setup(const gasfm_gatt_prob* in, int nprob, float* scratch, uint32_t* counters, bool bwd, GaArgs& a) {
+  const int resident = resident_blocks(
+      bwd ? reinterpret_cast<const void*>(&gatt_bwd_kernel) : reinterpret_cast<const void*>(&gatt_fwd_kernel), kT, 0);
   a.nprob = nprob;
+  int cap = resident;
+  for (int q = 0; q < nprob; ++q)
+    if (in[q].HC == H * 256) cap -= blocks_of(in[q].S, 256, 0);
+  const int most = bwd ? kMaxSlotsBwd : kMaxSlotsFwd;
+  cap = cap < most ? (cap < 1 ? 1 : cap) : most;
   int blocks = 0;
   float* ws = scratch;
   uint32_t* cn = counters;
@@ -613,19 +585,13 @@
     p.out = s.out, p.smax = s.smax, p.ssum = s.ssum, p.part = s.part;
     p.gout = s.gout, p.dXL = s.dXL, p.ldDXL = s.ldDXL, p.dXR = s.dXR, p.datt = s.datt;
     p.S = s.S, p.HC = s.HC, p.C = s.HC / H;
-    p.nblk = (s.S + chunk_of(p.C) - 1) / chunk_of(p.C);
-    if (p.nblk < 1) p.nblk = 1;
+    p.nblk = blocks_of(p.S, p.C, cap);
+    p.range = p.C == 256 ? kChunkV : range_of(p.S, p.nblk);
     p.blk0 = blocks;
     p.slots = ws;
     p.sl = p.HC + 2 * H;
-    const int64_t slot = bwd ? 2 * p.HC : p.HC + 2 * H;
-    ws += int64_t(p.nblk) * slot;
-    p.ngroups = groups_of(p.nblk);
-    p.gslots = ws;
-    if (p.ngroups > 1) ws += int64_t(p.ngroups) * slot;
+    ws += int64_t(p.nblk) * (bwd ? 2 * p.HC : p.HC + 2 * H);
     p.cnt = cn++;
-    p.gcnt = cn;
-    if (p.ngroups > 1) cn += p.ngroups;
     blocks += p.nblk;
   }
   for (int q = nprob; q < kMaxProb; ++q) a.p[q].blk0 = blocks;
@@ -647,45 +613,35 @@
     GASFM_REQUIRE(aligned16(p.XL) && aligned16(p.XR) && aligned16(p.att) && aligned16(p.bias),
                   "gasfm_gatt: problem %d alignment", q);
     if (!bwd) {
-      GASFM_REQUIRE(p.part || (p.out && p.smax && p.ssum), "gasfm_gatt_fwd: problem %d outputs", q);
+      GASFM_REQUIRE(p.part ? aligned16(p.part) : (p.out && p.smax && p.ssum), "gasfm_gatt_fwd: problem %d outputs", q);
     } else {
       GASFM_REQUIRE(p.gout && p.out && p.smax && p.ssum && (p.dXL || p.S == 0) && p.dXR && p.datt && p.ldDXL % 4 == 0 &&
-                        (aligned16(p.dXL) || p.S == 0) && aligned16(p.gout) && aligned16(p.out) && aligned16(p.datt),
+                        (aligned16(p.dXL) || p.S == 0) && aligned16(p.gout) && aligned16(p.out) && aligned16(p.datt) &&
+                        aligned16(p.dXR),
                     "gasfm_gatt_bwd: problem %d pointers", q);
     }
   }
   return GASFM_OK;
 }
 
-static int64_t nblk_of(const gasfm_gatt_prob& p) {
-  const int C = p.HC / H;
-  const int64_t nblk = (p.S + chunk_of(C) - 1) / chunk_of(C);
-  return nblk < 1 ? 1 : nblk;
-}
+static int64_t max_blocks_of(const gasfm_gatt_prob& p) { return blocks_of(p.S, p.HC / H, kMaxSlots); }
 
 extern "C" int64_t gasfm_gatt_scratch_floats(int32_t nprob, const gasfm_gatt_prob* probs) {
   int64_t n = 0;
-  for (int q = 0; q < nprob; ++q) {
-    const int64_t nblk = nblk_of(probs[q]), ng = groups_of(int(nblk));
-    n += (nblk + (ng > 1 ? ng : 0)) * (2 * int64_t(probs[q].HC) + 2 * H);
-  }
+  for (int q = 0; q < nprob; ++q) n += max_blocks_of(probs[q]) * (2 * int64_t(probs[q].HC) + 2 * H);
   return n + 16;
 }
 
 extern "C" int32_t gasfm_gatt_counters(int32_t nprob, const gasfm_gatt_prob* probs) {
-  int32_t n = 0;
-  for (int q = 0; q < nprob; ++q) {
-    const int ng = groups_of(int(nblk_of(probs[q])));
-    n += 1 + (ng > 1 ? ng : 0);
-  }
-  return n;
+  (void)probs;
+  return nprob;
 }
 
 extern "C" int gasfm_gatt_fwd(int32_t nprob, const gasfm_gatt_prob* probs, float slope, float* scratch,
                               uint32_t* counters, void* stream) {
   const int s0 = gatt_check(nprob, probs, false);
   if (s0 != GASFM_OK) return s0;
-  GASFM_REQUIRE(scratch && counters, "gasfm_gatt_fwd: scratch / counters");
+  GASFM_REQUIRE(scratch && counters && aligned16(scratch), "gasfm_gatt_fwd: scratch / counters");
   GaArgs a{};
   a.slope = slope;
   const int blocks = setup(probs, nprob, scratch, counters, false, a);
@@ -754,7 +710,7 @@
   for (int q = 0; q < nprob; ++q) {
     const gasfm_gatt_prob& s = probs[q];
     GASFM_REQUIRE((s.HC == 1024 || s.HC == 64) && s.part && s.bias && s.out && s.smax && s.ssum &&
-                      stride >= s.HC + 2 * H,
+                      stride >= s.HC + 2 * H && stride % 4 == 0 && aligned16(s.part),
                   "gasfm_gatt_merge: problem %d HC=%d / pointers / stride", q, s.HC);
     GaProb& p = a.p[q];
     p.HC = s.HC, p.C = s.HC / H, p.bias = s.bias, p.out = s.out, p.smax = s.smax, p.ssum = s.ssum;
@@ -762,7 +718,6 @@
     p.slots = const_cast<float*>(s.part);
     p.sl = stride;
     p.nblk = nrows;
-    p.ngroups = 1;
   }
   const int units = u.G ? (u.rows_dst ? u.m * (u.width / 4) : 0) + (u.sum_dst ? u.sn / 4 : 0) : 0;
   hipLaunchKernelGGL(gatt_merge_kernel, dim3(nprob + (units + kT - 1) / kT), dim3(kT), 0,
@@ -774,7 +729,7 @@
                               uint32_t* counters, void* stream) {
   const int s0 = gatt_check(nprob, probs, true);
   if (s0 != GASFM_OK) return s0;
-  GASFM_REQUIRE(scratch && counters, "gasfm_gatt_bwd: scratch / counters");
+  GASFM_REQUIRE(scratch && counters && aligned16(scratch), "gasfm_gatt_bwd: scratch / counters");
   GaArgs a{};
   a.slope = slope;
   const int blocks = setup(probs, nprob, scratch, counters, true, a);
```

Result: no change. 145.8 million edges/s, median of 6 (+0.9%).
